# William-gregory/SeaIceExtentForecasting

Hardware: NVIDIA B200
Metric: retrospective forecasts/sec (network+GPR) (higher is better)
Workload: dtype f64

## Files before the change

### include/sie_b200.h

```cpp
#ifndef SIE_B200_H
#define SIE_B200_H

#include <stddef.h>
#include <stdint.h>

#ifdef __cplusplus
extern "C" {
#endif

#define SIE_OK 0
#define SIE_ERR_ARG (-1)
#define SIE_ERR_LAUNCH (-2)
#define SIE_ERR_UNSUPPORTED (-3)

#define SIE_JOB_OK 0
#define SIE_JOB_NO_NAN_CELL 1
#define SIE_JOB_FEW_AREAS 2
#define SIE_JOB_CAPACITY 3

#define SIE_AREA_WORK 32

int sie_abi_version(void);
const char* sie_last_error(void);
int sie_device_info(int* sm_count, int* max_smem_optin, size_t* l2_bytes);

int sie_detrend_zscore(const double* fields, const int32_t* job_field, const int32_t* job_T,
                       int B, int C, int Tstride, int Tp, int do_detrend,
                       double* dt, double* trend, double* z,
                       int32_t* node_cell, int32_t* cell_node, int32_t* n_nodes,
                       int32_t* first_nan_cell, int32_t* status, int ldn, void* stream);

#define SIE_CORR_AUTO 0
#define SIE_CORR_TILES 1
#define SIE_CORR_ROWS 2
#define SIE_CORR_ROWS_MIRROR 3
#define SIE_CORR_TMA 4
int sie_corr_tau(const double* z, const int32_t* n_nodes, const int32_t* job_T, const double* r_crit,
                 int B, int ldn, int Tp, double* R,
                 double* tile_part, size_t tile_part_bytes,
                 double* tau_sum, int64_t* tau_cnt, double* tau,
                 int shard_rank, int shard_count, int kernel, void* stream);
size_t sie_corr_tau_scratch_bytes(int B, int ldn);

int sie_corr_rows(const double* z, const int32_t* rows, int n_rows, int N, int T, int Tp, double* out, int ld_out,
                  void* stream);

int sie_corr_stencil(const double* R, const double* z, const int32_t* job_T, int Tp,
                     const int32_t* node_cell, const int32_t* cell_node,
                     const int32_t* n_nodes, int B, int X, int Y, int ldn, int latlon,
                     double* stencil, void* stream);

int sie_area_level(const double* R, const double* z, const int32_t* job_T, int Tp,
                   const double* stencil, const int32_t* node_cell,
                   const int32_t* cell_node, const int32_t* n_nodes, const double* tau,
                   const int32_t* first_nan_cell, int B, int X, int Y, int ldn, int latlon,
                   int max_areas, int32_t* area_cells, int32_t* area_start, int32_t* area_key,
                   int32_t* n_areas, int32_t* label, int32_t* status,
                   void* scratch, size_t scratch_bytes, uint64_t* work, void* stream);
size_t sie_area_level_scratch_bytes(int B, int C);

int sie_intra_links(const double* dt, const double* scale, const int32_t* job_T,
                    const int32_t* area_cells, const int32_t* area_start, const int32_t* n_areas,
                    const int32_t* label, int B, int C, int Tstride, int max_areas,
                    double* anomaly, double* links, double* strength, double* strengthmap,
                    void* stream);

typedef struct SieGpProblem {
  int32_t job_sic;
  int32_t job_sst;
  int32_t n;
  int32_t y_off;
  int32_t rule;
  int32_t zscore;
  int32_t want_grad;
  int32_t pad_;
  double r_sel;
  double ell;
  double sig;
} SieGpProblem;

typedef struct SieGpResult {
  double fmean, fvar, sigma_f, nlml, g_ell, g_sig;
  int32_t n_pred, expm_m, expm_s, info;
  int64_t cycles_total, cycles_expm;
} SieGpResult;

int sie_gp_forecast(const SieGpProblem* prob, int P, const double* y_all,
                    const double* anom_sic, const int32_t* n_areas_sic, int max_areas_sic, int Tstride_sic,
                    const double* anom_sst, const int32_t* n_areas_sst, int max_areas_sst, int Tstride_sst,
                    int max_pred, SieGpResult* out, void* scratch, size_t scratch_bytes, void* stream);
size_t sie_gp_scratch_bytes(int P, int max_pred, int max_n);
int sie_debug_gp_phases(unsigned long long* out16);

int sie_gp_hyper_grid(const SieGpProblem* prob, int P, const double* sig_grid, int n_sig, const double* y_all,
                      const double* anom_sic, const int32_t* n_areas_sic, int max_areas_sic, int Tstride_sic,
                      const double* anom_sst, const int32_t* n_areas_sst, int max_areas_sst, int Tstride_sst,
                      int max_pred, SieGpResult* out, void* scratch, size_t scratch_bytes, void* stream);

int sie_nsidc_monthly(const uint8_t* files, int n_files, size_t file_stride, int header_bytes, int C,
                      double* monthly, void* stream);
int sie_polar_hole_fill(const double* monthly, const double* lat, double hole, int C, double* filled,
                        double* phole, double* scratch, void* stream);
int sie_regrid_linear(const double* src, int F, int C, const int32_t* vert, const double* bary, int Ct,
                      double* dst, void* stream);

#ifdef __cplusplus
}
#endif
#endif
```

### seaiceextentforecasting_b200/_lib.py

```python
from __future__ import annotations

import ctypes as C
import os

HERE = os.path.dirname(os.path.abspath(__file__))
LIB_PATH = os.path.join(HERE, "libsie_b200.so")

SIE_JOB_OK, SIE_JOB_NO_NAN_CELL, SIE_JOB_FEW_AREAS, SIE_JOB_CAPACITY = 0, 1, 2, 3
SIE_CORR_AUTO, SIE_CORR_TILES, SIE_CORR_ROWS, SIE_CORR_ROWS_MIRROR, SIE_CORR_TMA = 0, 1, 2, 3, 4
ABI_VERSION = 2
SIE_AREA_WORK = 32

c_i32 = C.c_int32
c_p = C.c_void_p
c_sz = C.c_size_t


class SieGpProblem(C.Structure):
    _fields_ = [("job_sic", c_i32), ("job_sst", c_i32), ("n", c_i32), ("y_off", c_i32), ("rule", c_i32),
                ("zscore", c_i32), ("want_grad", c_i32), ("pad_", c_i32), ("r_sel", C.c_double),
                ("ell", C.c_double), ("sig", C.c_double)]


class SieGpResult(C.Structure):
    _fields_ = [("fmean", C.c_double), ("fvar", C.c_double), ("sigma_f", C.c_double), ("nlml", C.c_double),
                ("g_ell", C.c_double), ("g_sig", C.c_double), ("n_pred", c_i32), ("expm_m", c_i32),
                ("expm_s", c_i32), ("info", c_i32), ("cycles_total", C.c_int64), ("cycles_expm", C.c_int64)]


_SIGS = {
    "sie_abi_version": (C.c_int, []),
    "sie_last_error": (C.c_char_p, []),
    "sie_device_info": (C.c_int, [C.POINTER(C.c_int), C.POINTER(C.c_int), C.POINTER(c_sz)]),
    "sie_detrend_zscore": (C.c_int, [c_p, c_p, c_p, C.c_int, C.c_int, C.c_int, C.c_int, C.c_int, c_p, c_p, c_p,
                                     c_p, c_p, c_p, c_p, c_p, C.c_int, c_p]),
    "sie_corr_tau": (C.c_int, [c_p, c_p, c_p, c_p, C.c_int, C.c_int, C.c_int, c_p, c_p, c_sz, c_p, c_p, c_p,
                               C.c_int, C.c_int, C.c_int, c_p]),
    "sie_corr_tau_scratch_bytes": (c_sz, [C.c_int, C.c_int]),
    "sie_corr_rows": (C.c_int, [c_p, c_p, C.c_int, C.c_int, C.c_int, C.c_int, c_p, C.c_int, c_p]),
    "sie_corr_stencil": (C.c_int, [c_p, c_p, c_p, C.c_int, c_p, c_p, c_p, C.c_int, C.c_int, C.c_int, C.c_int, C.c_int,
                                   c_p, c_p]),
    "sie_area_level": (C.c_int, [c_p, c_p, c_p, C.c_int, c_p, c_p, c_p, c_p, c_p, c_p, C.c_int, C.c_int, C.c_int,
                                 C.c_int, C.c_int, C.c_int, c_p, c_p, c_p, c_p, c_p, c_p, c_p, c_sz, c_p, c_p]),
    "sie_area_level_scratch_bytes": (c_sz, [C.c_int, C.c_int]),
    "sie_intra_links": (C.c_int, [c_p, c_p, c_p, c_p, c_p, c_p, c_p, C.c_int, C.c_int, C.c_int, C.c_int, c_p, c_p,
                                  c_p, c_p, c_p]),
    "sie_gp_forecast": (C.c_int, [c_p, C.c_int, c_p, c_p, c_p, C.c_int, C.c_int, c_p, c_p, C.c_int, C.c_int,
                                  C.c_int, c_p, c_p, c_sz, c_p]),
    "sie_gp_scratch_bytes": (c_sz, [C.c_int, C.c_int, C.c_int]),
    "sie_nsidc_monthly": (C.c_int, [c_p, C.c_int, c_sz, C.c_int, C.c_int, c_p, c_p]),
    "sie_polar_hole_fill": (C.c_int, [c_p, c_p, C.c_double, C.c_int, c_p, c_p, c_p, c_p]),
    "sie_regrid_linear": (C.c_int, [c_p, C.c_int, C.c_int, c_p, c_p, C.c_int, c_p, c_p]),
    "sie_gp_hyper_grid": (C.c_int, [c_p, C.c_int, c_p, C.c_int, c_p, c_p, c_p, C.c_int, C.c_int, c_p, c_p, C.c_int,
                                    C.c_int, C.c_int, c_p, c_p, c_sz, c_p]),
    "sie_debug_gp_phases": (C.c_int, [C.POINTER(C.c_ulonglong)]),
}

EXPORTED_SYMBOLS = tuple(_SIGS)
_lib = None


class SieError(RuntimeError):
    pass


def load():
    global _lib
    if _lib is not None:
        return _lib
    if not os.path.exists(LIB_PATH):
        raise SieError(f"{LIB_PATH} is missing: run `python -c 'import __graft_entry__ as g; g.build()'` "
                       "(the CUDA extension is the only implementation; there is no CPU fallback)")
    lib = C.CDLL(LIB_PATH)
    for name, (res, args) in _SIGS.items():
        fn = getattr(lib, name)
        fn.restype = res
        fn.argtypes = args
    if lib.sie_abi_version() != ABI_VERSION:
        raise SieError(f"{LIB_PATH} has ABI version {lib.sie_abi_version()}, this package needs {ABI_VERSION}: rebuild")
    _lib = lib
    return lib


def check(rc, what):
    if rc != 0:
        msg = load().sie_last_error()
        raise SieError(f"{what} failed (rc={rc}): {msg.decode() if msg else ''}")
```

### seaiceextentforecasting_b200/csrc/abi.cu

```cuda
#include <cstdarg>
#include <cstdio>
#include <mutex>
#include <cuda.h>
#include <cudaTypedefs.h>
#include "common.cuh"

static thread_local char g_err[512] = "";

void sie_set_error(const char* fmt, ...) {
  va_list ap;
  va_start(ap, fmt);
  vsnprintf(g_err, sizeof(g_err), fmt, ap);
  va_end(ap);
}

static SieDevice g_dev[SIE_MAX_DEVICES];
static std::mutex g_dev_mutex;

const SieDevice* sie_device(void) {
  int dev = 0;
  if (cudaGetDevice(&dev) != cudaSuccess || dev < 0 || dev >= SIE_MAX_DEVICES) {
    (void)cudaGetLastError();
    sie_set_error("no CUDA device (or device ordinal >= %d)", SIE_MAX_DEVICES);
    return nullptr;
  }
  SieDevice* d = &g_dev[dev];
  if (!d->ready) {
    std::lock_guard<std::mutex> lock(g_dev_mutex);
    if (!d->ready) {
      int v = 0;
      d->ordinal = dev;
      cudaDeviceGetAttribute(&v, cudaDevAttrMultiProcessorCount, dev); d->sm_count = v;
      cudaDeviceGetAttribute(&v, cudaDevAttrMaxSharedMemoryPerBlockOptin, dev); d->max_smem_optin = v;
      cudaDeviceGetAttribute(&v, cudaDevAttrMaxSharedMemoryPerMultiprocessor, dev); d->smem_per_sm = v;
      cudaDeviceGetAttribute(&v, cudaDevAttrL2CacheSize, dev); d->l2_bytes = (size_t)v;
      for (int i = 0; i < SIE_ATTR_SLOTS; ++i) d->attr_smem[i] = -1;
      d->ready = 1;
    }
  }
  return d;
}

int sie_ensure_smem(const SieDevice* d, int slot, const void* func, size_t bytes) {
  SieDevice* m = const_cast<SieDevice*>(d);
  if ((long long)bytes <= (long long)m->attr_smem[slot]) return SIE_OK;
  std::lock_guard<std::mutex> lock(g_dev_mutex);
  if ((long long)bytes <= (long long)m->attr_smem[slot]) return SIE_OK;
  if (cudaFuncSetAttribute(func, cudaFuncAttributeMaxDynamicSharedMemorySize, (int)bytes) != cudaSuccess) {
    sie_set_error("cudaFuncSetAttribute(%zu B of dynamic shared memory) failed: %s", bytes,
                  cudaGetErrorString(cudaGetLastError()));
    return SIE_ERR_LAUNCH;
  }
  m->attr_smem[slot] = (long long)bytes;
  return SIE_OK;
}

int sie_tensor_map_f64_3d(void* out, const double* base, int B, int ld, int box_cols, int box_rows) {
  static PFN_cuTensorMapEncodeTiled encode = nullptr;
  static std::once_flag once;
  std::call_once(once, [] {
    void* fn = nullptr;
    cudaDriverEntryPointQueryResult qres;
    if (cudaGetDriverEntryPoint("cuTensorMapEncodeTiled", &fn, cudaEnableDefault, &qres) == cudaSuccess &&
        qres == cudaDriverEntryPointSuccess)
      encode = reinterpret_cast<PFN_cuTensorMapEncodeTiled>(fn);
    else
      (void)cudaGetLastError();
  });
  if (!encode) {
    sie_set_error("cuTensorMapEncodeTiled is not available from this driver");
    return SIE_ERR_UNSUPPORTED;
  }
  const cuuint64_t dims[3] = {(cuuint64_t)ld, (cuuint64_t)ld, (cuuint64_t)B};
  const cuuint64_t strides[2] = {(cuuint64_t)ld * sizeof(double), (cuuint64_t)ld * (cuuint64_t)ld * sizeof(double)};
  const cuuint32_t box[3] = {(cuuint32_t)box_cols, (cuuint32_t)box_rows, 1u};
  const cuuint32_t estr[3] = {1u, 1u, 1u};
  const CUresult rc = encode(reinterpret_cast<CUtensorMap*>(out), CU_TENSOR_MAP_DATA_TYPE_FLOAT64, 3,
                             const_cast<double*>(base), dims, strides, box, estr, CU_TENSOR_MAP_INTERLEAVE_NONE,
                             CU_TENSOR_MAP_SWIZZLE_NONE, CU_TENSOR_MAP_L2_PROMOTION_NONE, CU_TENSOR_MAP_FLOAT_OOB_FILL_NONE);
  if (rc != CUDA_SUCCESS) {
    sie_set_error("cuTensorMapEncodeTiled failed (CUresult %d; B=%d ld=%d box=%dx%d)", (int)rc, B, ld, box_rows, box_cols);
    return SIE_ERR_LAUNCH;
  }
  return SIE_OK;
}

extern "C" int sie_abi_version(void) { return 2; }
extern "C" const char* sie_last_error(void) { return g_err; }

extern "C" int sie_device_info(int* sm_count, int* max_smem_optin, size_t* l2_bytes) {
  const SieDevice* d = sie_device();
  if (!d) return SIE_ERR_LAUNCH;
  if (sm_count) *sm_count = d->sm_count;
  if (max_smem_optin) *max_smem_optin = d->max_smem_optin;
  if (l2_bytes) *l2_bytes = d->l2_bytes;
  return SIE_OK;
}
```

### seaiceextentforecasting_b200/csrc/area.cu

```cuda
#include <type_traits>
#include "common.cuh"

#ifdef SIE_AREA_LDG
#define SIE_RLOAD(p) __ldg(p)
#else
#define SIE_RLOAD(p) __ldcg(p)
#endif

namespace {

constexpr int LEAF = 128;
constexpr int DCAP_MAX = 1024;
constexpr int MAXCH = 32;
constexpr unsigned long long NOKEY64 = ~0ull;
constexpr unsigned FULL = 0xffffffffu;

template <int NT_, typename IT_>
struct AreaCfg {
  static constexpr int NT = NT_;
  static constexpr int NW = NT_ / 32;
  static constexpr int NG = NT_ / 8;
  static constexpr int FCAP = NT_ >= 512 ? 256 : 192;
  static constexpr int BKW = NW - 1;
  static constexpr int CTAS = NT_ >= 512 ? 1 : 2;
  using IT = IT_;
  using FK = typename std::conditional<sizeof(IT_) == 2, uint16_t, uint32_t>::type;
  static constexpr FK NOKEY = (FK)~(FK)0;
  static constexpr int DSHIFT = sizeof(IT_) == 2 ? 14 : 28;
  static_assert(FCAP <= NT - 32, "slot threads and the bookkeeping warp must be distinct");
};

enum : int { PL_LAB = 1, PL_FKEY = 2, PL_FLIST = 4, PL_HN = 8, PL_HC = 16, PL_CNL = 32, PL_KNL = 64, PL_AREA = 128 };

__host__ __device__ inline size_t align_up(size_t x, size_t a) { return (x + a - 1) / a * a; }
__host__ __device__ inline size_t rm_cap(int C) { return (size_t)4 * C + 1024 + 256; }
__host__ __device__ inline int d_cap(int C) { return C < DCAP_MAX ? C : DCAP_MAX; }
__host__ __device__ inline size_t area_tab_bytes(int MA, size_t isz) {
  return 12 * align_up(isz * (size_t)(MA + 1), 16) + 2 * align_up(sizeof(double) * (size_t)MA, 16);
}
__host__ __device__ inline size_t self_cap(int C) { return (size_t)2 * C + 64; }
__host__ __device__ inline size_t slot_bytes(int fcap) { return sizeof(double) * (18 * (size_t)fcap) + sizeof(int32_t) * 2 * (size_t)fcap; }
constexpr size_t QUEUE_BYTES = 256;
__host__ __device__ inline size_t scratch_per_cta(int C, int MA) {
  size_t s = 0;
  s += align_up(sizeof(int32_t) * (size_t)C, 256);
  s += align_up(sizeof(int32_t) * (size_t)7 * C, 256);
  s += align_up(sizeof(double) * rm_cap(C), 256);
  s += align_up(sizeof(double) * ((size_t)d_cap(C) * d_cap(C) + 128), 256);
  s += align_up(area_tab_bytes(MA, sizeof(int32_t)), 256);
  s += align_up(sizeof(double) * (self_cap(C) + 256), 256);
  return s;
}

template <typename IT>
struct AreaTabs {
  IT *a_start, *a_len, *seg_next, *tail, *size, *fin, *nlist;
  IT *xoff, *xep, *xrows;
  IT *self_off, *self_sz;
  unsigned long long* okey;
  double* stat;
};
template <typename IT>
__device__ inline AreaTabs<IT> carve_tabs(unsigned char* p, int MA) {
  AreaTabs<IT> t;
  auto take = [&](size_t bytes) { unsigned char* r = p; p += align_up(bytes, 16); return r; };
  t.a_start = (IT*)take(sizeof(IT) * (size_t)(MA + 1));
  t.a_len = (IT*)take(sizeof(IT) * (size_t)(MA + 1));
  t.seg_next = (IT*)take(sizeof(IT) * (size_t)(MA + 1));
  t.tail = (IT*)take(sizeof(IT) * (size_t)(MA + 1));
  t.size = (IT*)take(sizeof(IT) * (size_t)(MA + 1));
  t.fin = (IT*)take(sizeof(IT) * (size_t)(MA + 1));
  t.nlist = (IT*)take(sizeof(IT) * (size_t)(MA + 1));
  t.xoff = (IT*)take(sizeof(IT) * (size_t)(MA + 1));
  t.xep = (IT*)take(sizeof(IT) * (size_t)(MA + 1));
  t.xrows = (IT*)take(sizeof(IT) * (size_t)(MA + 1));
  t.self_off = (IT*)take(sizeof(IT) * (size_t)(MA + 1));
  t.self_sz = (IT*)take(sizeof(IT) * (size_t)(MA + 1));
  t.okey = (unsigned long long*)take(sizeof(double) * (size_t)MA);
  t.stat = (double*)take(sizeof(double) * (size_t)MA);
  return t;
}

struct Rec {
  unsigned long long ord, pri;
  uint32_t a, b;
};
__device__ __forceinline__ Rec rec_none() { Rec r; r.ord = 0ull; r.pri = 0ull; r.a = 0u; r.b = 0u; return r; }
__device__ __forceinline__ unsigned long long ord_of(double x) {
  x = __dadd_rn(x, 0.0);
  const unsigned long long u = (unsigned long long)__double_as_longlong(x);
  return (u >> 63) ? ~u : (u | 0x8000000000000000ull);
}
__device__ __forceinline__ double ord_to_double(unsigned long long o) {
  const unsigned long long u = (o >> 63) ? (o & 0x7fffffffffffffffull) : ~o;
  return __longlong_as_double((long long)u);
}
__device__ __forceinline__ Rec rec_max(const Rec& x, const Rec& y) {
  const bool ty = (y.ord > x.ord) || (y.ord == x.ord && y.pri > x.pri);
  return ty ? y : x;
}
template <int PW>
__device__ __forceinline__ Rec warp_arg(const Rec& r) {
  const uint32_t w0 = (uint32_t)(r.ord >> 32), w1 = (uint32_t)r.ord;
  const uint32_t w2 = (uint32_t)(r.pri >> 32), w3 = (uint32_t)r.pri;
  const uint32_t m0 = __reduce_max_sync(FULL, w0);
  bool ok = (w0 == m0);
  {
    const unsigned b0 = __ballot_sync(FULL, ok);
    if ((b0 & (b0 - 1u)) == 0u) {
      const int src0 = __ffs(b0) - 1;
      Rec o;
      o.ord = ((unsigned long long)m0 << 32) | __shfl_sync(FULL, w1, src0);
      o.pri = ((unsigned long long)__shfl_sync(FULL, w2, src0) << 32) | __shfl_sync(FULL, w3, src0);
      o.a = __shfl_sync(FULL, r.a, src0);
      o.b = __shfl_sync(FULL, r.b, src0);
      return o;
    }
  }
  const uint32_t m1 = __reduce_max_sync(FULL, ok ? w1 : 0u);
  ok = ok && (w1 == m1);
  const uint32_t m2 = __reduce_max_sync(FULL, ok ? w2 : 0u);
// ... 82 lines not shown
  if (diag) return sie_nan();
  double acc = 0.0;
  for (int k = 0; k < kT; k += 4) {
    const double2 a0 = *reinterpret_cast<const double2*>(za + k), a1 = *reinterpret_cast<const double2*>(za + k + 2);
    const double2 c0 = *reinterpret_cast<const double2*>(zc + k), c1 = *reinterpret_cast<const double2*>(zc + k + 2);
    acc = fma(a0.x, c0.x, acc);
    acc = fma(a0.y, c0.y, acc);
    acc = fma(a1.x, c1.x, acc);
    acc = fma(a1.y, c1.y, acc);
  }
  if (!(fabs(acc) <= 1.0)) acc = acc > 1.0 ? 1.0 : (acc < -1.0 ? -1.0 : acc);
  return acc;
}

template <class CFG, bool ONCHIP, bool ZR>
__global__ void __launch_bounds__(CFG::NT, CFG::CTAS)
k_area_level(const double* __restrict__ Rall, const int32_t* __restrict__ job_T, int Tp,
             const double* __restrict__ stencil_all,
             const int32_t* __restrict__ node_cell_all, const int32_t* __restrict__ cell_node_all,
             const int32_t* __restrict__ n_nodes, const double* __restrict__ tau_all,
             const int32_t* __restrict__ first_nan_cell, int B, int X, int Y, int ldn, int latlon, int MA,
             int32_t* __restrict__ area_cells_all, int32_t* __restrict__ area_start_all,
             int32_t* __restrict__ area_key_all, int32_t* __restrict__ n_areas_all,
             int32_t* __restrict__ label_all, int32_t* __restrict__ status_all,
             int* __restrict__ queue, unsigned char* __restrict__ scratch_all, size_t scratch_stride, int place_arg,
             unsigned long long* __restrict__ work_all) {
  constexpr int NT = CFG::NT, NW = CFG::NW, NG = CFG::NG, FCAP = CFG::FCAP, BKW = CFG::BKW;
  using IT = typename CFG::IT;
  using FK = typename CFG::FK;
  constexpr FK NOKEY = CFG::NOKEY;
  constexpr int MAXD = ONCHIP ? 6 : 16;
  const int place = ONCHIP ? 0 : place_arg;
  extern __shared__ __align__(16) unsigned char smem_raw[];
  __shared__ RecSlot rslots[2 * NW];
  __shared__ int sh_i[8];
  __shared__ int sh_koff[MAXCH + 1], sh_uoff[MAXCH + 1];
  __shared__ int sh_goff[MAXCH + 1], sh_soff[MAXCH + 1], sh_xo[MAXCH], sh_r0[MAXCH], sh_so[MAXCH];
  __shared__ int sh_x[4];
  __shared__ int sh_job;
  __shared__ unsigned long long sh_work;
  __shared__ unsigned long long ph[16];
  long long tick_last = 0;
#ifdef SIE_AREA_PHASE_TIMERS
#define TICK(i)                                                        \
  do {                                                                 \
    if (tid == 0) {                                                    \
      const long long t__ = clock64();                                 \
      ph[i] += (unsigned long long)(t__ - tick_last);                  \
      tick_last = t__;                                                 \
    }                                                                  \
  } while (0)
#else
#define TICK(i) do { } while (0)
#endif
  long long btick = 0;
#ifdef SIE_AREA_PHASE_TIMERS
#define BTICK(i)                                                       \
  do {                                                                 \
    const long long t__ = clock64();                                   \
    bph[i] += (unsigned long long)(t__ - btick);                       \
    btick = t__;                                                       \
  } while (0)
#else
#define BTICK(i) do { } while (0)
#endif

  const int tid = threadIdx.x, lane = tid & 31, warp = tid >> 5;
  const int g = tid >> 3, j = tid & 7;
  const unsigned gmask = 0xffu << (lane & 24);
  const int C = X * Y;
  int par = 0;

  unsigned char* gp = scratch_all + (size_t)blockIdx.x * scratch_stride;
  auto gtake = [&](size_t bytes) { unsigned char* r = gp; gp += align_up(bytes, 256); return r; };
  int32_t* s1_cells = (int32_t*)gtake(sizeof(int32_t) * (size_t)C);
  IT* ibuf = (IT*)gtake(sizeof(int32_t) * (size_t)7 * C);
  double* rowmean = (double*)gtake(sizeof(double) * rm_cap(C));
  const int dcap = d_cap(C);
  double* D = (double*)gtake(sizeof(double) * ((size_t)dcap * dcap + 128));
  unsigned char* gtabs = gtake(area_tab_bytes(MA, sizeof(int32_t)));
  double* selfbuf = (double*)gtake(sizeof(double) * (self_cap(C) + 256));
  unsigned char* sp = smem_raw;
  auto stake = [&](size_t bytes) { unsigned char* r = sp; sp += align_up(bytes, 16); return r; };
  double* facc = (double*)stake(sizeof(double) * 8 * FCAP);
  double* ftail = (double*)stake(sizeof(double) * 8 * FCAP);
  double* sres = (double*)stake(sizeof(double) * FCAP);
  double* smean = (double*)stake(sizeof(double) * FCAP);
  int32_t* snan = (int32_t*)stake(sizeof(int32_t) * FCAP);
  int32_t* srow = (int32_t*)stake(sizeof(int32_t) * FCAP);
  AreaTabs<IT> S = carve_tabs<IT>((place & PL_AREA) ? gtabs : stake(area_tab_bytes(MA, sizeof(IT))), MA);
  auto iarr = [&](int bit, int idx) -> IT* {
    return (place & bit) ? ibuf + (size_t)idx * C : (IT*)stake(sizeof(IT) * (size_t)C);
  };
  IT* lab = iarr(PL_LAB, 0);
  FK* fkey = (FK*)iarr(PL_FKEY, 1);
  IT* flist = iarr(PL_FLIST, 2);
  IT* hn = iarr(PL_HN, 3);
  IT* hc = iarr(PL_HC, 4);
  IT* cnl = iarr(PL_CNL, 5);
  IT* knl = iarr(PL_KNL, 6);
  const IT* cnode = cnl;

  for (;;) {
  __syncthreads();
  if (tid == 0) sh_job = atomicAdd(queue, 1);
  __syncthreads();
  const int b = sh_job;
  if (b >= B) break;
  unsigned long long wk = 0;
#ifdef SIE_AREA_PHASE_TIMERS
  unsigned long long rbucket[6] = {0, 0, 0, 0, 0, 0};
#endif
  unsigned long long bph[8] = {0, 0, 0, 0, 0, 0, 0, 0};
  const int N = min(n_nodes[b], ldn);
  const double tau = tau_all[b];
  const double* R = ZR ? Rall + (size_t)b * ldn * Tp : Rall + (size_t)b * ldn * ldn;
  const int kT = ZR ? ((job_T[b] + 3) & ~3) : 0;
  const RCtx rcx = {R, ldn, Tp, kT};
  struct RowH { const double* p; int n; };
  auto rrow = [&](int a) -> RowH { RowH h; h.n = a; h.p = R + (size_t)a * (ZR ? Tp : ldn); return h; };
  auto rat = [&](const RowH& h, int c) -> double {
    if constexpr (ZR) return sie_zcorr(h.p, R + (size_t)c * Tp, kT, h.n == c);
    else if constexpr (sizeof(IT) == 2) return SIE_RLOAD(R + (unsigned)(min(c, h.n) * ldn + max(c, h.n)));
    else return (c >= h.n) ? SIE_RLOAD(h.p + c) : SIE_RLOAD(R + (size_t)c * ldn + h.n);
  };
  const double* sten = stencil_all + (size_t)b * ldn * 4;
  const int32_t* cnode_g = cell_node_all + (size_t)b * C;
  int32_t* out_cells = area_cells_all + (size_t)b * C;
  int32_t* out_start = area_start_all + (size_t)b * (MA + 1);
  int32_t* out_key = area_key_all + (size_t)b * MA;
  int32_t* out_label = label_all + (size_t)b * C;

  for (int c = tid; c < C; c += NT) { lab[c] = -1; fkey[c] = NOKEY; out_label[c] = -1; cnl[c] = (IT)cnode_g[c]; }
  if (tid < 16) ph[tid] = 0ull;
  if (tid == 0) { n_areas_all[b] = 0; out_start[0] = 0; sh_work = 0ull; if (work_all) work_all[SIE_AREA_WORK * b] = 0ull; }
  __syncthreads();
  if (first_nan_cell[b] < 0) {
    if (tid == 0) status_all[b] = SIE_JOB_NO_NAN_CELL;
    continue;
  }
  if (status_all[b] == SIE_JOB_CAPACITY) continue;

  auto init_slot = [&](int s, int fnode, int n) {
    const RowH row = rrow(fnode);
    const int ngrp = n >> 3, nt = n & 7;
    double r, tv;
    int nanc = 0;
    sie_pw_lane8_any([&](int i) { return rat(row, hn[i]); }, 0, n, ngrp, nt, j, r, tv, nanc);
    facc[j * FCAP + s] = r;
    ftail[j * FCAP + s] = tv;
    double res = 0.0;
    if (ngrp > 0) {
      res = __dadd_rn(r, __shfl_xor_sync(gmask, r, 1));
      res = __dadd_rn(res, __shfl_xor_sync(gmask, res, 2));
      res = __dadd_rn(res, __shfl_xor_sync(gmask, res, 4));
    }
    res = sie_add_tail8(res, tv, nt, gmask);
    nanc += __shfl_xor_sync(gmask, nanc, 1);
    nanc += __shfl_xor_sync(gmask, nanc, 2);
    nanc += __shfl_xor_sync(gmask, nanc, 4);
    if (j == 0) {
      sres[s] = res;
      snan[s] = nanc;
      srow[s] = fnode;
      smean[s] = res / (double)(n - nanc);
    }
  };
  auto bk_add = [&](int m, int p, int nmem, int hole, int nf, bool do_init, bool& fits) -> int {
    bool isnew = false;
    int f = -1;
    if (lane < 4) {
      const int d = lane;
      const int ci = m / Y, cj = m - ci * Y;
      const int a = ci + (d == 0 ? -1 : (d == 1 ? 1 : 0));
      const int q = cj + (d == 2 ? -1 : (d == 3 ? 1 : 0));
      if (a >= 0 && a < X && q >= 0 && q < Y) {
        f = a * Y + q;
        const int fn = cnode[f];
        if (lab[f] >= 0 || fn < 0 || fn >= N) f = -1;
      }
      if (f >= 0) {
        const FK key = (FK)(((uint32_t)d << CFG::DSHIFT) | (uint32_t)p);
        const FK old = fkey[f];
// ... 482 lines not shown
      }
      if (off > xtop) { ++epoch; xtop = ld; }
      extend_D(nb, off);
      nb = off;
    } else {
      if (tid == 0) S.fin[best] = 1;
    }
    __syncthreads();
    TICK(12);
#ifdef SIE_AREA_PHASE_TIMERS
    if (tid == 0) {
      const int bk = round_nb0 <= 4 ? 0 : round_nb0 <= 8 ? 1 : round_nb0 <= 16 ? 2 : round_nb0 <= 32 ? 3 : round_nb0 <= 64 ? 4 : 5;
      rbucket[bk] += (1ull << 44) + (unsigned long long)(clock64() - round_t0);
    }
#endif
  }

  if (wk) atomicAdd(&sh_work, wk);
  __syncthreads();
  if (tid == 0 && work_all) {
    const long long clk2 = clock64();
    work_all[SIE_AREA_WORK * b] = sh_work;
    work_all[SIE_AREA_WORK * b + 1] = (unsigned long long)(clk1 - clk0);
    work_all[SIE_AREA_WORK * b + 2] = (unsigned long long)(clk2 - clk1);
    work_all[SIE_AREA_WORK * b + 3] = (n_steps << 32) | n_rounds;
    for (int i = 0; i < 11; ++i) work_all[SIE_AREA_WORK * b + 4 + i] = ph[i];
    work_all[SIE_AREA_WORK * b + 24] = ph[11];
    work_all[SIE_AREA_WORK * b + 25] = ph[12];
#ifdef SIE_AREA_PHASE_TIMERS
    for (int i = 0; i < 6; ++i) work_all[SIE_AREA_WORK * b + 26 + i] = rbucket[i];
#endif
    work_all[SIE_AREA_WORK * b + 15] = n_slow;
  }
  if (tid == BKW * 32 && work_all)
    for (int i = 0; i < 8; ++i) work_all[SIE_AREA_WORK * b + 16 + i] = bph[i];
  if (tid == 0) {
    int cnt = 0, off = 0;
    for (int k = 0; k < nA; ++k) {
      if (S.size[k] > 0) {
        out_key[cnt] = k;
        out_start[cnt] = off;
        S.nlist[cnt] = (IT)k;
        off += S.size[k];
        ++cnt;
      }
    }
    out_start[cnt] = off;
    n_areas_all[b] = cnt;
    status_all[b] = (cnt < 2) ? SIE_JOB_FEW_AREAS : SIE_JOB_OK;
    sh_i[4] = cnt;
  }
  __syncthreads();
  const int cnt = sh_i[4];
  for (int a = 0; a < cnt; ++a) {
    int off = out_start[a];
    for (int s = S.nlist[a]; s >= 0; s = S.seg_next[s]) {
      const int st = S.a_start[s], ln = S.a_len[s];
      for (int i = tid; i < ln; i += NT) {
        const int c = s1_cells[st + i];
        out_cells[off + i] = c;
        out_label[c] = a;
      }
      off += ln;
    }
  }
  }
}

template <class CFG, bool ONCHIP, bool ZR>
int launch_area(const SieDevice* dev, int slot, int grid, size_t smem, cudaStream_t st, const double* R,
                const int32_t* job_T, int Tp, const double* stencil, const int32_t* node_cell, const int32_t* cell_node, const int32_t* n_nodes,
                const double* tau, const int32_t* first_nan_cell, int B, int X, int Y, int ldn, int latlon,
                int max_areas, int32_t* area_cells, int32_t* area_start, int32_t* area_key, int32_t* n_areas,
                int32_t* label, int32_t* status, int* queue, unsigned char* scratch, size_t per_cta, int place,
                unsigned long long* work) {
  auto kern = k_area_level<CFG, ONCHIP, ZR>;
  if (int rc = sie_ensure_smem(dev, slot, (const void*)kern, smem)) return rc;
  kern<<<grid, CFG::NT, smem, st>>>(R, job_T, Tp, stencil, node_cell, cell_node, n_nodes, tau, first_nan_cell, B, X, Y, ldn, latlon,
                                    max_areas, area_cells, area_start, area_key, n_areas, label, status, queue, scratch,
                                    per_cta, place, work);
  return SIE_OK;
}

struct AreaPlan { int variant, ctas_per_sm, place; size_t smem; };
AreaPlan plan_area(const SieDevice* dev, int B, int C, int ldn, int max_areas, bool force32 = false) {
  AreaPlan pl = {2, 1, 0, 0};
  const size_t budget = (size_t)dev->max_smem_optin - 4096;
  if (!force32 && C < 8192 && ldn <= 32767 && max_areas <= 32766) {
    const size_t i16 = 7 * align_up(sizeof(int16_t) * (size_t)C, 16) + area_tab_bytes(max_areas, sizeof(int16_t)) + 64;
    const size_t s256 = align_up(slot_bytes(AreaCfg<256, int16_t>::FCAP), 16) + i16;
    const size_t s512 = align_up(slot_bytes(AreaCfg<512, int16_t>::FCAP), 16) + i16;
    const int sms = dev->sm_count;
    const double t512 = (double)((B + sms - 1) / sms);
    const double t256 = (double)((B + 2 * sms - 1) / (2 * sms)) * (B > sms ? 1.64 : 1.3);
    if (t256 < t512 && 2 * (s256 + 4096 + 1024) <= (size_t)dev->smem_per_sm) {
      pl.variant = 0; pl.ctas_per_sm = 2; pl.smem = s256; return pl;
    }
    if (s512 <= budget) { pl.variant = 1; pl.smem = s512; return pl; }
  }
  const size_t ibytes = align_up(sizeof(int32_t) * (size_t)C, 16);
  const size_t tabs = area_tab_bytes(max_areas, sizeof(int32_t));
  size_t smem = align_up(slot_bytes(AreaCfg<512, int32_t>::FCAP), 16) + 64 + tabs + 7 * ibytes;
  const int order[8] = {PL_KNL, PL_AREA, PL_HC, PL_FLIST, PL_HN, PL_FKEY, PL_CNL, PL_LAB};
  for (int i = 0; i < 8 && smem > budget; ++i) {
    pl.place |= order[i];
    smem -= (order[i] == PL_AREA) ? tabs : ibytes;
  }
  pl.smem = smem;
  return pl;
}

}

extern "C" size_t sie_area_level_scratch_bytes(int B, int C) {
  const SieDevice* dev = sie_device();
  const int sms = (dev && dev->sm_count > 0) ? dev->sm_count : 148;
  const int g = B < 2 * sms ? (B > 0 ? B : 1) : 2 * sms;
  return QUEUE_BYTES + (size_t)g * scratch_per_cta(C, C / 2 + 1);
}

extern "C" int sie_area_level(const double* R, const double* z, const int32_t* job_T, int Tp, const double* stencil,
                              const int32_t* node_cell, const int32_t* cell_node, const int32_t* n_nodes,
                              const double* tau, const int32_t* first_nan_cell, int B, int X, int Y, int ldn, int latlon,
                              int max_areas, int32_t* area_cells, int32_t* area_start, int32_t* area_key,
                              int32_t* n_areas, int32_t* label, int32_t* status, void* scratch,
                              size_t scratch_bytes, uint64_t* work, void* stream) {
  SIE_CHECK_ARG(stencil && node_cell && cell_node && n_nodes && tau && first_nan_cell && area_cells &&
                    area_start && area_key && n_areas && label && status && scratch, "null pointer");
  SIE_CHECK_ARG(R || (z && job_T && Tp >= 4 && (Tp % 4) == 0), "without R the unit-norm rows z, job_T and Tp are needed");
  SIE_CHECK_ARG(B > 0 && X > 0 && Y > 0 && ldn > 0 && max_areas > 0, "non-positive size");
  const int C = X * Y;
  SIE_CHECK_ARG(max_areas <= C / 2 + 1, "max_areas cannot exceed C/2+1");
  SIE_CHECK_ARG((long long)C < (1ll << 22), "grid too large (frontier key encoding / pairwise tree depth)");
  const SieDevice* dev = sie_device();
  if (!dev) return SIE_ERR_LAUNCH;
  const bool zr = (R == nullptr);
  const AreaPlan pl = plan_area(dev, B, C, ldn, max_areas, zr);
  SIE_CHECK_ARG(pl.smem <= (size_t)dev->max_smem_optin - 4096, "shared memory budget");
  const size_t per_cta = scratch_per_cta(C, max_areas);
  SIE_CHECK_ARG(scratch_bytes >= QUEUE_BYTES + per_cta, "scratch too small");
  long long grid = (long long)pl.ctas_per_sm * dev->sm_count;
  if (grid > B) grid = B;
  const long long fit = (long long)((scratch_bytes - QUEUE_BYTES) / per_cta);
  if (grid > fit) grid = fit;
  cudaStream_t st = (cudaStream_t)stream;
  int* queue = reinterpret_cast<int*>(scratch);
  unsigned char* blocks = reinterpret_cast<unsigned char*>(scratch) + QUEUE_BYTES;
  if (cudaMemsetAsync(queue, 0, sizeof(int), st) != cudaSuccess) SIE_CHECK_LAUNCH();
  int rc;
#define SIE_AREA_ARGS                                                                                                   \
  job_T, Tp, stencil, node_cell, cell_node, n_nodes, tau, first_nan_cell, B, X, Y, ldn, latlon, max_areas, area_cells,   \
      area_start, area_key, n_areas, label, status, queue, blocks, per_cta, pl.place, (unsigned long long*)work
  const bool on32 = (pl.place == 0 && C < 8192);
  if (zr && on32)
    rc = launch_area<AreaCfg<512, int32_t>, true, true>(dev, SIE_K_AREA_ON32_Z, (int)grid, pl.smem, st, z, SIE_AREA_ARGS);
  else if (zr)
    rc = launch_area<AreaCfg<512, int32_t>, false, true>(dev, SIE_K_AREA_OFF32_Z, (int)grid, pl.smem, st, z, SIE_AREA_ARGS);
  else if (pl.variant == 0)
    rc = launch_area<AreaCfg<256, int16_t>, true, false>(dev, SIE_K_AREA_ON16_2, (int)grid, pl.smem, st, R, SIE_AREA_ARGS);
  else if (pl.variant == 1)
    rc = launch_area<AreaCfg<512, int16_t>, true, false>(dev, SIE_K_AREA_ON16, (int)grid, pl.smem, st, R, SIE_AREA_ARGS);
  else if (on32)
    rc = launch_area<AreaCfg<512, int32_t>, true, false>(dev, SIE_K_AREA_ON32, (int)grid, pl.smem, st, R, SIE_AREA_ARGS);
  else
    rc = launch_area<AreaCfg<512, int32_t>, false, false>(dev, SIE_K_AREA_OFF32, (int)grid, pl.smem, st, R, SIE_AREA_ARGS);
#undef SIE_AREA_ARGS
  if (rc) return rc;
  SIE_CHECK_LAUNCH();
  return SIE_OK;
}
```

### seaiceextentforecasting_b200/csrc/common.cuh

```cuda
#pragma once
#include <cuda_runtime.h>
#include <stdint.h>
#include <math.h>
#include "../../include/sie_b200.h"

void sie_set_error(const char* fmt, ...);

#define SIE_MAX_DEVICES 64
#define SIE_ATTR_SLOTS 16
enum SieAttrSlot { SIE_K_DETREND = 0, SIE_K_CORR_TILES, SIE_K_CORR_ROWS_ST, SIE_K_CORR_ROWS_MIR, SIE_K_CORR_ROWS_TAU, SIE_K_AREA_ON32,
                   SIE_K_AREA_OFF32, SIE_K_AREA_ON16, SIE_K_AREA_ON16_2, SIE_K_AREA_ON32_Z, SIE_K_AREA_OFF32_Z, SIE_K_GP,
                   SIE_K_LINKS, SIE_K_CORR_TMA };
struct SieDevice {
  volatile int ready;
  int ordinal, sm_count, max_smem_optin, smem_per_sm;
  size_t l2_bytes;
  long long attr_smem[SIE_ATTR_SLOTS];
};
const SieDevice* sie_device(void);
int sie_ensure_smem(const SieDevice* d, int slot, const void* func, size_t bytes);
int sie_tensor_map_f64_3d(void* out128, const double* base, int B, int ld, int box_cols, int box_rows);

#define SIE_CHECK_ARG(cond, msg)                 \
  do {                                           \
    if (!(cond)) {                               \
      sie_set_error("%s: %s", __func__, msg);    \
      return SIE_ERR_ARG;                        \
    }                                            \
  } while (0)

#define SIE_CHECK_LAUNCH()                                                   \
  do {                                                                       \
    cudaError_t e__ = cudaGetLastError();                                    \
    if (e__ != cudaSuccess) {                                                \
      sie_set_error("%s: CUDA error %s", __func__, cudaGetErrorString(e__)); \
      return SIE_ERR_LAUNCH;                                                 \
    }                                                                        \
  } while (0)

__device__ __forceinline__ double sie_nan() { return __longlong_as_double(0x7ff8000000000000LL); }

#ifndef SIE_PW_SMALL_NQ
#define SIE_PW_SMALL_NQ 8
#endif
template <int NQ> __device__ __forceinline__ void sie_fence_regs(double (&v)[NQ]);
template <> __device__ __forceinline__ void sie_fence_regs<1>(double (&v)[1]) { asm volatile("" : "+d"(v[0])); }
template <> __device__ __forceinline__ void sie_fence_regs<4>(double (&v)[4]) {
  asm volatile("" : "+d"(v[0]), "+d"(v[1]), "+d"(v[2]), "+d"(v[3]));
}
template <> __device__ __forceinline__ void sie_fence_regs<8>(double (&v)[8]) {
  asm volatile("" : "+d"(v[0]), "+d"(v[1]), "+d"(v[2]), "+d"(v[3]), "+d"(v[4]), "+d"(v[5]), "+d"(v[6]), "+d"(v[7]));
}
template <> __device__ __forceinline__ void sie_fence_regs<6>(double (&v)[6]) {
  asm volatile("" : "+d"(v[0]), "+d"(v[1]), "+d"(v[2]), "+d"(v[3]), "+d"(v[4]), "+d"(v[5]));
}
template <> __device__ __forceinline__ void sie_fence_regs<10>(double (&v)[10]) {
  asm volatile("" : "+d"(v[0]), "+d"(v[1]), "+d"(v[2]), "+d"(v[3]), "+d"(v[4]), "+d"(v[5]), "+d"(v[6]), "+d"(v[7]),
                    "+d"(v[8]), "+d"(v[9]));
}
template <> __device__ __forceinline__ void sie_fence_regs<12>(double (&v)[12]) {
  asm volatile("" : "+d"(v[0]), "+d"(v[1]), "+d"(v[2]), "+d"(v[3]), "+d"(v[4]), "+d"(v[5]), "+d"(v[6]), "+d"(v[7]),
                    "+d"(v[8]), "+d"(v[9]), "+d"(v[10]), "+d"(v[11]));
}
template <> __device__ __forceinline__ void sie_fence_regs<16>(double (&v)[16]) {
  asm volatile("" : "+d"(v[0]), "+d"(v[1]), "+d"(v[2]), "+d"(v[3]), "+d"(v[4]), "+d"(v[5]), "+d"(v[6]), "+d"(v[7]),
                    "+d"(v[8]), "+d"(v[9]), "+d"(v[10]), "+d"(v[11]), "+d"(v[12]), "+d"(v[13]), "+d"(v[14]), "+d"(v[15]));
}

__device__ __forceinline__ double sie_add_tail8(double res, double tv, int nt, unsigned gmask) {
  double t[7];
#pragma unroll
  for (int i = 0; i < 7; ++i) t[i] = __shfl_sync(gmask, tv, i, 8);
#pragma unroll
  for (int i = 0; i < 7; ++i) if (i < nt) res = __dadd_rn(res, t[i]);
  return res;
}

template <int NQ, typename Get>
__device__ __forceinline__ void sie_pw_lane8(Get get, int lo, int n, int ngrp, int ntail, int j, double& acc, double& tv,
                                             int& nan_cnt) {
  double v[NQ];
#pragma unroll
  for (int k = 0; k < NQ; ++k) v[k] = get(lo + min(8 * k + j, n - 1));
  double t[1];
  t[0] = get(lo + min(8 * ngrp + j, n - 1));
  sie_fence_regs<NQ>(v);
  sie_fence_regs<1>(t);
  tv = t[0];
  if (j >= ntail) tv = 0.0;
  if (tv != tv) { tv = 0.0; ++nan_cnt; }
  double r = 0.0;
#pragma unroll
  for (int k = 0; k < NQ; ++k) {
    if (k < ngrp) {
      double x = v[k];
      if (x != x) { x = 0.0; ++nan_cnt; }
      r = (k == 0) ? x : __dadd_rn(r, x);
    }
  }
  acc = r;
// ... 128 lines not shown
```

Before: 67530.

## Add compact 3-CTA/SM area-level variant with occupancy-checked cost-model planner

Result: faster. 70230, median of 6 (+4.0%).

```diff
diff --git a/include/sie_b200.h b/include/sie_b200.h
--- a/include/sie_b200.h
+++ b/include/sie_b200.h
@@ -58,6 +58,7 @@
                    int32_t* n_areas, int32_t* label, int32_t* status,
                    void* scratch, size_t scratch_bytes, uint64_t* work, void* stream);
 size_t sie_area_level_scratch_bytes(int B, int C);
+int sie_area_level_plan(int B, int C, int ldn, int max_areas, int* variant, int* ctas_per_sm);
 
 int sie_intra_links(const double* dt, const double* scale, const int32_t* job_T,
                     const int32_t* area_cells, const int32_t* area_start, const int32_t* n_areas,
diff --git a/seaiceextentforecasting_b200/_lib.py b/seaiceextentforecasting_b200/_lib.py
--- a/seaiceextentforecasting_b200/_lib.py
+++ b/seaiceextentforecasting_b200/_lib.py
@@ -43,6 +43,7 @@
     "sie_area_level": (C.c_int, [c_p, c_p, c_p, C.c_int, c_p, c_p, c_p, c_p, c_p, c_p, C.c_int, C.c_int, C.c_int,
                                  C.c_int, C.c_int, C.c_int, c_p, c_p, c_p, c_p, c_p, c_p, c_p, c_sz, c_p, c_p]),
     "sie_area_level_scratch_bytes": (c_sz, [C.c_int, C.c_int]),
+    "sie_area_level_plan": (C.c_int, [C.c_int, C.c_int, C.c_int, C.c_int, C.POINTER(C.c_int), C.POINTER(C.c_int)]),
     "sie_intra_links": (C.c_int, [c_p, c_p, c_p, c_p, c_p, c_p, c_p, C.c_int, C.c_int, C.c_int, C.c_int, c_p, c_p,
                                   c_p, c_p, c_p]),
     "sie_gp_forecast": (C.c_int, [c_p, C.c_int, c_p, c_p, c_p, C.c_int, C.c_int, c_p, c_p, C.c_int, C.c_int,
diff --git a/seaiceextentforecasting_b200/csrc/abi.cu b/seaiceextentforecasting_b200/csrc/abi.cu
--- a/seaiceextentforecasting_b200/csrc/abi.cu
+++ b/seaiceextentforecasting_b200/csrc/abi.cu
@@ -34,7 +34,7 @@
       cudaDeviceGetAttribute(&v, cudaDevAttrMaxSharedMemoryPerBlockOptin, dev); d->max_smem_optin = v;
       cudaDeviceGetAttribute(&v, cudaDevAttrMaxSharedMemoryPerMultiprocessor, dev); d->smem_per_sm = v;
       cudaDeviceGetAttribute(&v, cudaDevAttrL2CacheSize, dev); d->l2_bytes = (size_t)v;
-      for (int i = 0; i < SIE_ATTR_SLOTS; ++i) d->attr_smem[i] = -1;
+      for (int i = 0; i < SIE_ATTR_SLOTS; ++i) { d->attr_smem[i] = -1; d->occ[i] = -1; }
       d->ready = 1;
     }
   }
diff --git a/seaiceextentforecasting_b200/csrc/area.cu b/seaiceextentforecasting_b200/csrc/area.cu
--- a/seaiceextentforecasting_b200/csrc/area.cu
+++ b/seaiceextentforecasting_b200/csrc/area.cu
@@ -1,3 +1,4 @@
+#include <algorithm>
 #include <type_traits>
 #include "common.cuh"
 
@@ -15,28 +16,37 @@
 constexpr unsigned long long NOKEY64 = ~0ull;
 constexpr unsigned FULL = 0xffffffffu;
 
-template <int NT_, typename IT_>
+template <int NT_, typename IT_, int FCAP_, int CTAS_, bool COMPACT_ = false>
 struct AreaCfg {
   static constexpr int NT = NT_;
   static constexpr int NW = NT_ / 32;
   static constexpr int NG = NT_ / 8;
-  static constexpr int FCAP = NT_ >= 512 ? 256 : 192;
+  static constexpr int FCAP = FCAP_;
   static constexpr int BKW = NW - 1;
-  static constexpr int CTAS = NT_ >= 512 ? 1 : 2;
+  static constexpr int CTAS = CTAS_;
+  static constexpr bool COMPACT = COMPACT_;
   using IT = IT_;
   using FK = typename std::conditional<sizeof(IT_) == 2, uint16_t, uint32_t>::type;
   static constexpr FK NOKEY = (FK)~(FK)0;
   static constexpr int DSHIFT = sizeof(IT_) == 2 ? 14 : 28;
   static_assert(FCAP <= NT - 32, "slot threads and the bookkeeping warp must be distinct");
 };
+using CfgP3 = AreaCfg<160, int16_t, 128, 3, true>;
+using CfgP2 = AreaCfg<256, int16_t, 192, 2>;
+using CfgM16 = AreaCfg<512, int16_t, 256, 1>;
+using CfgL32 = AreaCfg<512, int32_t, 256, 1>;
+constexpr int AREA_MAX_CTAS_PER_SM = 3;
 
 enum : int { PL_LAB = 1, PL_FKEY = 2, PL_FLIST = 4, PL_HN = 8, PL_HC = 16, PL_CNL = 32, PL_KNL = 64, PL_AREA = 128 };
 
 __host__ __device__ inline size_t align_up(size_t x, size_t a) { return (x + a - 1) / a * a; }
 __host__ __device__ inline size_t rm_cap(int C) { return (size_t)4 * C + 1024 + 256; }
 __host__ __device__ inline int d_cap(int C) { return C < DCAP_MAX ? C : DCAP_MAX; }
+__host__ __device__ inline size_t area_int_tab_bytes(int MA, size_t isz) {
+  return 12 * align_up(isz * (size_t)(MA + 1), 16);
+}
 __host__ __device__ inline size_t area_tab_bytes(int MA, size_t isz) {
-  return 12 * align_up(isz * (size_t)(MA + 1), 16) + 2 * align_up(sizeof(double) * (size_t)MA, 16);
+  return area_int_tab_bytes(MA, isz) + 2 * align_up(sizeof(double) * (size_t)MA, 16);
 }
 __host__ __device__ inline size_t self_cap(int C) { return (size_t)2 * C + 64; }
 __host__ __device__ inline size_t slot_bytes(int fcap) { return sizeof(double) * (18 * (size_t)fcap) + sizeof(int32_t) * 2 * (size_t)fcap; }
@@ -285,23 +295,45 @@
   double* selfbuf = (double*)gtake(sizeof(double) * (self_cap(C) + 256));
   unsigned char* sp = smem_raw;
   auto stake = [&](size_t bytes) { unsigned char* r = sp; sp += align_up(bytes, 16); return r; };
-  double* facc = (double*)stake(sizeof(double) * 8 * FCAP);
-  double* ftail = (double*)stake(sizeof(double) * 8 * FCAP);
-  double* sres = (double*)stake(sizeof(double) * FCAP);
-  double* smean = (double*)stake(sizeof(double) * FCAP);
-  int32_t* snan = (int32_t*)stake(sizeof(int32_t) * FCAP);
-  int32_t* srow = (int32_t*)stake(sizeof(int32_t) * FCAP);
-  AreaTabs<IT> S = carve_tabs<IT>((place & PL_AREA) ? gtabs : stake(area_tab_bytes(MA, sizeof(IT))), MA);
   auto iarr = [&](int bit, int idx) -> IT* {
     return (place & bit) ? ibuf + (size_t)idx * C : (IT*)stake(sizeof(IT) * (size_t)C);
   };
-  IT* lab = iarr(PL_LAB, 0);
-  FK* fkey = (FK*)iarr(PL_FKEY, 1);
-  IT* flist = iarr(PL_FLIST, 2);
-  IT* hn = iarr(PL_HN, 3);
-  IT* hc = iarr(PL_HC, 4);
-  IT* cnl = iarr(PL_CNL, 5);
-  IT* knl = iarr(PL_KNL, 6);
+  double *facc, *ftail, *sres, *smean;
+  int32_t *snan, *srow;
+  auto take_slots = [&]() {
+    facc = (double*)stake(sizeof(double) * 8 * FCAP);
+    ftail = (double*)stake(sizeof(double) * 8 * FCAP);
+    sres = (double*)stake(sizeof(double) * FCAP);
+    smean = (double*)stake(sizeof(double) * FCAP);
+    snan = (int32_t*)stake(sizeof(int32_t) * FCAP);
+    srow = (int32_t*)stake(sizeof(int32_t) * FCAP);
+  };
+  AreaTabs<IT> S;
+  IT *lab, *hn, *cnl, *hc, *knl;
+  FK* fkey;
+  IT* flist;
+  if constexpr (CFG::COMPACT) {
+    S = carve_tabs<IT>(stake(area_int_tab_bytes(MA, sizeof(IT))), MA);
+    const AreaTabs<IT> G = carve_tabs<IT>(gtabs, MA);
+    S.okey = G.okey;
+    S.stat = G.stat;
+    lab = iarr(0, 0); hn = iarr(0, 3); cnl = iarr(0, 5);
+    unsigned char* const phase = sp;
+    take_slots();
+    fkey = (FK*)iarr(0, 1); flist = iarr(0, 2);
+    sp = phase;
+    hc = iarr(0, 4); knl = iarr(0, 6);
+  } else {
+    take_slots();
+    S = carve_tabs<IT>((place & PL_AREA) ? gtabs : stake(area_tab_bytes(MA, sizeof(IT))), MA);
+    lab = iarr(PL_LAB, 0);
+    fkey = (FK*)iarr(PL_FKEY, 1);
+    flist = iarr(PL_FLIST, 2);
+    hn = iarr(PL_HN, 3);
+    hc = iarr(PL_HC, 4);
+    cnl = iarr(PL_CNL, 5);
+    knl = iarr(PL_KNL, 6);
+  }
   const IT* cnode = cnl;
 
   for (;;) {
@@ -950,25 +982,75 @@
   return SIE_OK;
 }
 
+template <class CFG>
+size_t area_smem_bytes(int C, int MA) {
+  const size_t isz = sizeof(typename CFG::IT), ib = align_up(isz * (size_t)C, 16), slots = align_up(slot_bytes(CFG::FCAP), 16);
+  if (CFG::COMPACT) return area_int_tab_bytes(MA, isz) + 3 * ib + std::max(slots + 2 * ib, 2 * ib) + 64;
+  return slots + area_tab_bytes(MA, isz) + 7 * ib + 64;
+}
+
 struct AreaPlan { int variant, ctas_per_sm, place; size_t smem; };
+template <class CFG>
+bool area_resident(const SieDevice* dev, int slot, size_t smem) {
+  SieDevice* m = const_cast<SieDevice*>(dev);
+  const long long key = (long long)smem << 8;
+  const long long hit = m->occ[slot];
+  if (hit >= 0 && (hit & ~255ll) == key) return (int)(hit & 255) >= CFG::CTAS;
+  auto kern = k_area_level<CFG, true, false>;
+  int n = 0;
+  if (sie_ensure_smem(dev, slot, (const void*)kern, smem) != SIE_OK) {
+    sie_set_error("%s", "");
+    n = 0;
+  } else if (cudaOccupancyMaxActiveBlocksPerMultiprocessor(&n, kern, CFG::NT, smem) != cudaSuccess) {
+    (void)cudaGetLastError();
+    n = 0;
+  }
+  m->occ[slot] = key | std::min(n, 255);
+  return n >= CFG::CTAS;
+}
 AreaPlan plan_area(const SieDevice* dev, int B, int C, int ldn, int max_areas, bool force32 = false) {
   AreaPlan pl = {2, 1, 0, 0};
   const size_t budget = (size_t)dev->max_smem_optin - 4096;
   if (!force32 && C < 8192 && ldn <= 32767 && max_areas <= 32766) {
-    const size_t i16 = 7 * align_up(sizeof(int16_t) * (size_t)C, 16) + area_tab_bytes(max_areas, sizeof(int16_t)) + 64;
-    const size_t s256 = align_up(slot_bytes(AreaCfg<256, int16_t>::FCAP), 16) + i16;
-    const size_t s512 = align_up(slot_bytes(AreaCfg<512, int16_t>::FCAP), 16) + i16;
+    struct Cand {
+      int variant, k, slot, min_waves;
+      size_t smem;
+      double f[3];
+      bool (*resident)(const SieDevice*, int, size_t);
+    };
+    const Cand cands[3] = {
+        {1, 1, SIE_K_AREA_ON16, 1, area_smem_bytes<CfgM16>(C, max_areas), {1.0, 1.0, 1.0}, area_resident<CfgM16>},
+        {0, 2, SIE_K_AREA_ON16_2, 1, area_smem_bytes<CfgP2>(C, max_areas), {1.18, 1.31, 1.31}, area_resident<CfgP2>},
+        {3, 3, SIE_K_AREA_ON16_3, 2, area_smem_bytes<CfgP3>(C, max_areas), {1.37, 1.47, 1.69}, area_resident<CfgP3>},
+    };
     const int sms = dev->sm_count;
-    const double t512 = (double)((B + sms - 1) / sms);
-    const double t256 = (double)((B + 2 * sms - 1) / (2 * sms)) * (B > sms ? 1.64 : 1.3);
-    if (t256 < t512 && 2 * (s256 + 4096 + 1024) <= (size_t)dev->smem_per_sm) {
-      pl.variant = 0; pl.ctas_per_sm = 2; pl.smem = s256; return pl;
-    }
-    if (s512 <= budget) { pl.variant = 1; pl.smem = s512; return pl; }
+    bool tried[3] = {false, false, false};
+    for (;;) {
+      int bi = -1;
+      double best = 0.0;
+      for (int i = 0; i < 3; ++i) {
+        const Cand& c = cands[i];
+#ifdef SIE_AREA_VARIANT
+        if (c.variant != SIE_AREA_VARIANT) continue;
+#endif
+        if (tried[i] || c.smem > budget) continue;
+        const long long waves = (B + (long long)c.k * sms - 1) / ((long long)c.k * sms);
+        if (waves < c.min_waves) continue;
+        const int s = std::min(c.k, (B + sms - 1) / sms);
+        const double t = (double)waves * c.f[s - 1];
+        if (bi < 0 || t < best) { bi = i; best = t; }
+      }
+      if (bi < 0) break;
+      tried[bi] = true;
+      const Cand& c = cands[bi];
+      if (c.k == 1 || c.resident(dev, c.slot, c.smem)) {
+        pl.variant = c.variant; pl.ctas_per_sm = c.k; pl.smem = c.smem; return pl;
+      }
+    }
   }
   const size_t ibytes = align_up(sizeof(int32_t) * (size_t)C, 16);
   const size_t tabs = area_tab_bytes(max_areas, sizeof(int32_t));
-  size_t smem = align_up(slot_bytes(AreaCfg<512, int32_t>::FCAP), 16) + 64 + tabs + 7 * ibytes;
+  size_t smem = align_up(slot_bytes(CfgL32::FCAP), 16) + 64 + tabs + 7 * ibytes;
   const int order[8] = {PL_KNL, PL_AREA, PL_HC, PL_FLIST, PL_HN, PL_FKEY, PL_CNL, PL_LAB};
   for (int i = 0; i < 8 && smem > budget; ++i) {
     pl.place |= order[i];
@@ -978,13 +1060,32 @@
   return pl;
 }
 
+int area_max_ctas_per_sm(const SieDevice* dev, int C) {
+  if (C >= 8192) return 1;
+  if (area_resident<CfgP3>(dev, SIE_K_AREA_ON16_3, area_smem_bytes<CfgP3>(C, 1))) return 3;
+  if (area_resident<CfgP2>(dev, SIE_K_AREA_ON16_2, area_smem_bytes<CfgP2>(C, 1))) return 2;
+  return 1;
+}
+
 }
 
 extern "C" size_t sie_area_level_scratch_bytes(int B, int C) {
   const SieDevice* dev = sie_device();
   const int sms = (dev && dev->sm_count > 0) ? dev->sm_count : 148;
-  const int g = B < 2 * sms ? (B > 0 ? B : 1) : 2 * sms;
+  const int cap = (dev ? area_max_ctas_per_sm(dev, C) : AREA_MAX_CTAS_PER_SM) * sms;
+  const int g = B < cap ? (B > 0 ? B : 1) : cap;
   return QUEUE_BYTES + (size_t)g * scratch_per_cta(C, C / 2 + 1);
+}
+
+extern "C" int sie_area_level_plan(int B, int C, int ldn, int max_areas, int* variant, int* ctas_per_sm) {
+  SIE_CHECK_ARG(variant && ctas_per_sm, "null pointer");
+  SIE_CHECK_ARG(B > 0 && C > 0 && ldn > 0 && max_areas > 0, "non-positive size");
+  const SieDevice* dev = sie_device();
+  if (!dev) return SIE_ERR_LAUNCH;
+  const AreaPlan pl = plan_area(dev, B, C, ldn, max_areas);
+  *variant = pl.variant;
+  *ctas_per_sm = pl.ctas_per_sm;
+  return SIE_OK;
 }
 
 extern "C" int sie_area_level(const double* R, const double* z, const int32_t* job_T, int Tp, const double* stencil,
@@ -1021,17 +1122,19 @@
       area_start, area_key, n_areas, label, status, queue, blocks, per_cta, pl.place, (unsigned long long*)work
   const bool on32 = (pl.place == 0 && C < 8192);
   if (zr && on32)
-    rc = launch_area<AreaCfg<512, int32_t>, true, true>(dev, SIE_K_AREA_ON32_Z, (int)grid, pl.smem, st, z, SIE_AREA_ARGS);
+    rc = launch_area<CfgL32, true, true>(dev, SIE_K_AREA_ON32_Z, (int)grid, pl.smem, st, z, SIE_AREA_ARGS);
   else if (zr)
-    rc = launch_area<AreaCfg<512, int32_t>, false, true>(dev, SIE_K_AREA_OFF32_Z, (int)grid, pl.smem, st, z, SIE_AREA_ARGS);
+    rc = launch_area<CfgL32, false, true>(dev, SIE_K_AREA_OFF32_Z, (int)grid, pl.smem, st, z, SIE_AREA_ARGS);
+  else if (pl.variant == 3)
+    rc = launch_area<CfgP3, true, false>(dev, SIE_K_AREA_ON16_3, (int)grid, pl.smem, st, R, SIE_AREA_ARGS);
   else if (pl.variant == 0)
-    rc = launch_area<AreaCfg<256, int16_t>, true, false>(dev, SIE_K_AREA_ON16_2, (int)grid, pl.smem, st, R, SIE_AREA_ARGS);
+    rc = launch_area<CfgP2, true, false>(dev, SIE_K_AREA_ON16_2, (int)grid, pl.smem, st, R, SIE_AREA_ARGS);
   else if (pl.variant == 1)
-    rc = launch_area<AreaCfg<512, int16_t>, true, false>(dev, SIE_K_AREA_ON16, (int)grid, pl.smem, st, R, SIE_AREA_ARGS);
+    rc = launch_area<CfgM16, true, false>(dev, SIE_K_AREA_ON16, (int)grid, pl.smem, st, R, SIE_AREA_ARGS);
   else if (on32)
-    rc = launch_area<AreaCfg<512, int32_t>, true, false>(dev, SIE_K_AREA_ON32, (int)grid, pl.smem, st, R, SIE_AREA_ARGS);
+    rc = launch_area<CfgL32, true, false>(dev, SIE_K_AREA_ON32, (int)grid, pl.smem, st, R, SIE_AREA_ARGS);
   else
-    rc = launch_area<AreaCfg<512, int32_t>, false, false>(dev, SIE_K_AREA_OFF32, (int)grid, pl.smem, st, R, SIE_AREA_ARGS);
+    rc = launch_area<CfgL32, false, false>(dev, SIE_K_AREA_OFF32, (int)grid, pl.smem, st, R, SIE_AREA_ARGS);
 #undef SIE_AREA_ARGS
   if (rc) return rc;
   SIE_CHECK_LAUNCH();
diff --git a/seaiceextentforecasting_b200/csrc/common.cuh b/seaiceextentforecasting_b200/csrc/common.cuh
--- a/seaiceextentforecasting_b200/csrc/common.cuh
+++ b/seaiceextentforecasting_b200/csrc/common.cuh
@@ -10,12 +10,13 @@
 #define SIE_ATTR_SLOTS 16
 enum SieAttrSlot { SIE_K_DETREND = 0, SIE_K_CORR_TILES, SIE_K_CORR_ROWS_ST, SIE_K_CORR_ROWS_MIR, SIE_K_CORR_ROWS_TAU, SIE_K_AREA_ON32,
                    SIE_K_AREA_OFF32, SIE_K_AREA_ON16, SIE_K_AREA_ON16_2, SIE_K_AREA_ON32_Z, SIE_K_AREA_OFF32_Z, SIE_K_GP,
-                   SIE_K_LINKS, SIE_K_CORR_TMA };
+                   SIE_K_LINKS, SIE_K_CORR_TMA, SIE_K_AREA_ON16_3 };
 struct SieDevice {
   volatile int ready;
   int ordinal, sm_count, max_smem_optin, smem_per_sm;
   size_t l2_bytes;
   long long attr_smem[SIE_ATTR_SLOTS];
+  long long occ[SIE_ATTR_SLOTS];
 };
 const SieDevice* sie_device(void);
 int sie_ensure_smem(const SieDevice* d, int slot, const void* func, size_t bytes);
```
